# interactiveaudiolab/emphases

Hardware: AMD Instinct MI355X
Metric: utterances/s (10 s @16 kHz) whole-node (higher is better)
Workload: dtype f32; 1 GPU; 64 synthetic 10 s 16 kHz utterances per GPU, conv config, random word alignments, ragged batch with per-utterance (B=1) semantics (BASELINE.json configs[1]); utterances_per_gpu=64, frames_per_gpu=64000, words_per_gpu=1882, conv_tile=64, launch=hipGraph replay, batches_in_flight=2, parallelism=utterance-sharded x1, exchange=none (one rank)

## Files before the change

### emphases_amd/csrc/forward.hip

```cpp
#include "common.h"

using namespace emph;

namespace emph {
__global__ __launch_bounds__(64) void launch_probe_kernel() {}
}

extern "C" {

int emph_launch_probe(void* stream) {
    EMPH_LAUNCH(launch_probe_kernel, dim3(1), dim3(64), 0, static_cast<hipStream_t>(stream));
    return check_launch("emph_launch_probe");
}

int64_t emph_prominence_workspace_floats(int32_t features, int32_t channels,
                                         int64_t ld_frames, int64_t ld_words,
                                         int32_t n_slots) {
    return (static_cast<int64_t>(features) + 2 * channels) * ld_frames +
           static_cast<int64_t>(channels) * (ld_words + n_slots);
}

int emph_prominence_forward(const emph_conv_model* model, const void* audio,
                            int32_t audio_format, const int64_t* seg,
                            const int32_t* frontend_tiles,
// ... 19 lines not shown
                 "emph_prominence_forward: conv_variant %d", m.conv_variant);
    EMPH_REQUIRE(!quad || tile_n == 64, EMPH_ERANGE,
                 "emph_prominence_forward: F(4,3) takes 64-position tiles, not %d", tile_n);
    const int64_t lds_square = quad ? emph_conv_winograd4_lds_bytes(m.channels, m.channels)
                                    : emph_conv_winograd_lds_bytes(m.channels, m.channels);
    const int64_t lds_input = quad ? emph_conv_winograd4_lds_bytes(m.channels, m.features)
                                   : emph_conv_winograd_lds_bytes(m.channels, m.features);
    EMPH_REQUIRE(lds_square <= 160 * 1024 && lds_input <= 160 * 1024, EMPH_ERANGE,
                 "emph_prominence_forward: %d channels do not fit the Winograd kernel's LDS",
                 m.channels);
    const int c = m.channels;
    float* features = workspace;
    float* current = features + static_cast<int64_t>(m.features) * ld_frames;
    float* other = current + static_cast<int64_t>(c) * ld_frames;
    float* words = other + static_cast<int64_t>(c) * ld_frames;
    float* sums = words + static_cast<int64_t>(c) * ld_words;
    const bool fold = word_sums != nullptr && m.encoder_layers > 0;
    EMPH_REQUIRE(!fold || (quad && (m.reduction == EMPH_REDUCE_SUM ||
                                    m.reduction == EMPH_REDUCE_AVERAGE)),
                 EMPH_EINVAL,
                 "emph_prominence_forward: word_sums needs conv_variant 1 and a sum / average "
                 "reduction");

    int status = emph_logmel(audio, audio_format, seg, frontend_tiles, n_frontend_tiles, m.table,
                             m.mel_start, m.mel_count, m.mel_offset, m.mel_values, m.mel_nnz,
                             features, ld_frames, 0, -1, nullptr, nullptr, m.normalize, stream);
    if (status) return status;
    auto conv = [&](const float* in, float* out, const float* pack, const float* bias, int c_in,
                    int activation) {
        return quad ? emph_conv1d_winograd4(in, ld_frames, out, ld_frames, pack, bias, c_in, c,
                                            activation, frame_tiles, n_frame_tiles, stream)
                    : emph_conv1d_winograd(in, ld_frames, out, ld_frames, pack, bias, c_in, c,
                                           activation, frame_tiles, n_frame_tiles, tile_n,
                                           stream);
    };
    const int64_t pack_floats =
        quad ? emph_conv_winograd4_pack_size(c, c) : emph_conv_winograd_pack_size(c, c);
    const bool stack = conv_spans != nullptr && quad && c == 80 && m.features == 80 &&
                       m.encoder_packs == m.input_pack + pack_floats &&
                       m.encoder_biases == m.input_bias + c &&
                       (m.activation == EMPH_ACT_RELU || m.activation == EMPH_ACT_NONE);
    if (stack) {
        const bool composed = m.compose != nullptr && m.encoder_layers >= 1;
        const int skip = composed ? 1 : 0;
        const int total = 1 + m.encoder_layers - skip;
        const int most = emph_conv_stack_max_layers();
        const int groups = (total + most - 1) / most;
        float* buffers[2] = {current, other};
        const float* in = features;
// ... 66 lines not shown
```

### emphases_amd/csrc/frontend.hip

```cpp
#include <math.h>
#include <stdarg.h>

#include "common.h"

namespace emph {

namespace {
thread_local char g_error[512] = "";
}

void set_error(const char* format, ...) {
    va_list args;
    va_start(args, format);
    vsnprintf(g_error, sizeof(g_error), format, args);
    va_end(args);
}

__device__ __forceinline__ void frontend_fence() {
    asm volatile("" ::: "memory");
    __builtin_amdgcn_wave_barrier();
}

__device__ __forceinline__ void frontend_section() { __builtin_amdgcn_sched_barrier(0); }

constexpr float kLn2 = 0.69314718055994530942f;
constexpr int kWaveFrames = 8;
constexpr int kPair = 1;
constexpr int kWavesPerSimd = 3;
constexpr int kTileStride = kWaveFrames + 1;
constexpr int kExRow = 72;
constexpr int kExRowB = 88;
constexpr int kExStepB = 9;
constexpr int kExFloats = 2 * 8 * kExRowB;
__device__ __forceinline__ int spectrum_slot(int k) { return k + 4 * (k >> 5); }
constexpr int kHighBase = 256 + 4 * (256 >> 5);
constexpr int kMagFloats = 560;
constexpr int kWaveFloats = kPair * kExFloats + kMels * kTileStride + kWaveFrames;
constexpr int kRunA = 24;
constexpr int kRunB = 12;

constexpr int kTabWindow = 0;
constexpr int kTabTw1 = 1024;
constexpr int kTabTw2 = kTabTw1 + 2 * 512;
constexpr int kTabTw3 = kTabTw2 + 2 * 64;
constexpr int kTabSize = kTabTw3 + 2 * 514;

typedef float cf __attribute__((ext_vector_type(2)));

template <int STRIDE>
__device__ __forceinline__ void lds_read8(cf (&v)[8], const cf* base) {
    const uint32_t address = static_cast<uint32_t>(reinterpret_cast<uintptr_t>(
        (const __attribute__((address_space(3))) cf*)base));
    asm volatile(
        "ds_read_b64 %0, %8\n\t"
        "ds_read_b64 %1, %8 offset:%9\n\t"
        "ds_read_b64 %2, %8 offset:%10\n\t"
        "ds_read_b64 %3, %8 offset:%11\n\t"
        "ds_read_b64 %4, %8 offset:%12\n\t"
        "ds_read_b64 %5, %8 offset:%13\n\t"
        "ds_read_b64 %6, %8 offset:%14\n\t"
// ... 155 lines not shown
__device__ __forceinline__ void load_edge(const Chunk& chunk, int frame, int p, cf (&s)[8]) {
    const int first = frame * kHop - kPad;
    const int safe = chunk.r_hi > chunk.r_lo ? chunk.r_lo : 0;
#pragma unroll
    for (int q = 0; q < 8; ++q) {
        float pair[2];
#pragma unroll
        for (int h = 0; h < 2; ++h) {
            int r = first + 2 * (p + 64 * q) + h;
            if (r < 0) r = -r;
            if (r >= chunk.length) r = 2 * (chunk.length - 1) - r;
            const bool live = r >= chunk.r_lo && r < chunk.r_hi;
            const int at = live ? r : safe;
            float value = 0.f;
            if (chunk.r_hi > chunk.r_lo)
                value = PCM ? static_cast<float>(static_cast<const int16_t*>(chunk.origin)[at])
                            : static_cast<const float*>(chunk.origin)[at];
            pair[h] = live ? value : 0.f;
        }
        s[q] = {pair[0], pair[1]};
    }
}

template <int MODE, bool PCM>
__global__ __launch_bounds__(256)
__attribute__((amdgpu_waves_per_eu(kWavesPerSimd, kWavesPerSimd))) void frontend_kernel(
    const void* __restrict__ audio, const int64_t* __restrict__ seg,
    const int32_t* __restrict__ tiles, const float* __restrict__ table,
    const int32_t* __restrict__ mel_start, const int32_t* __restrict__ mel_count,
    const int32_t* __restrict__ mel_offset, const float* __restrict__ mel_values,
    int mel_nnz, float* __restrict__ out, int64_t ld, int mel_row, int loud_row,
    float* __restrict__ seg_peak, const float* __restrict__ a_weights,
    int normalize, int n_tiles) {
    constexpr bool kMel = MODE == 0 || MODE == 2;
    constexpr bool kLoud = MODE == 2 || MODE == 3;
    constexpr bool kPeak = MODE == 1;
    constexpr float kPowerFloor = MODE == 0 ? 1e-6f : 0.f;

    extern __shared__ __align__(16) float lds[];
    const int tid = threadIdx.x;
    const int lane = tid & 63;
    const int wave = __builtin_amdgcn_readfirstlane(tid >> 6);
    float* mine = lds + wave * kWaveFloats;
    float* exchange = mine;
    float* tile = exchange + kPair * kExFloats;
    float* loud_tile = tile + kMels * kTileStride;
    float* weights = lds + 4 * kWaveFloats;

    if (kLoud) {
        for (int index = tid; index < kBins; index += 256) weights[index] = a_weights[index];
        __syncthreads();
    }

    const int p = lane;
    const int r1 = lane >> 3;
    const int p0 = lane & 7;
    float window[16];
    cf tw1[8], tw2[8], tw3[4];
#pragma unroll
    for (int q = 0; q < 8; ++q) {
        const float unit = PCM ? 1.f / 32768.f : 1.f;
        window[2 * q] = unit * table[kTabWindow + 2 * (p + 64 * q)];
        window[2 * q + 1] = unit * table[kTabWindow + 2 * (p + 64 * q) + 1];
        tw1[q] = {table[kTabTw1 + 2 * (q * 64 + p)],
                  table[kTabTw1 + 2 * (q * 64 + p) + 1]};
        tw2[q] = {table[kTabTw2 + 2 * (q * 8 + p0)],
                  table[kTabTw2 + 2 * (q * 8 + p0) + 1]};
    }
#pragma unroll
    for (int u = 0; u < 4; ++u) {
        const int k = r1 + 8 * p0 + 64 * u;
        tw3[u] = {table[kTabTw3 + 2 * k + 1], -table[kTabTw3 + 2 * k]};
    }
    auto bin_of = [&](int j) {
        const int k = r1 + 8 * p0 + 64 * (j & 3);
        return j == 8 ? 256 : (j < 4 ? k : 512 - k);
    };

    float weight_a[kRunA], weight_b[kRunB];
    int start_a = 0, start_b = 0;
    if (kMel) {
        const int first_a = mel_start[lane];
        const int count_a = mel_count[lane];
        const int offset_a = mel_offset[lane];
        start_a = first_a & ~3;
#pragma unroll
        for (int j = 0; j < kRunA; ++j) {
            const int index = start_a + j - first_a;
            weight_a[j] = (index >= 0 && index < count_a)
                              ? mel_values[min(max(offset_a + index, 0), mel_nnz - 1)]
                              : 0.f;
        }
        const int row_b = 64 + (lane >> 2);
        const int first_b = mel_start[row_b];
        const int count_b = mel_count[row_b];
        const int offset_b = mel_offset[row_b];
        start_b = (first_b & ~3) + kRunB * (lane & 3);
#pragma unroll
        for (int j = 0; j < kRunB; ++j) {
            const int index = start_b + j - first_b;
            weight_b[j] = (index >= 0 && index < count_b)
                              ? mel_values[min(max(offset_b + index, 0), mel_nnz - 1)]
                              : 0.f;
        }
// ... 142 lines not shown
                    db = fmaxf(db, floor_db) + weights[k];
                    total += static_cast<double>(fmaxf(db, -100.f));
                }
#pragma unroll
                for (int offset = 32; offset > 0; offset >>= 1)
                    total += __shfl_xor(total, offset);
                if (lane == 0) {
                    float value = static_cast<float>(total / 513.);
                    if (normalize) value = (value + 100.f) / 100.f;
                    loud_tile[min(local + f, valid - 1)] = value;
                }
            }
        }

        if (kMel) {
#pragma unroll
            for (int f = 0; f < kPair; ++f) {
                float* mag = exchange + f * kExFloats;
#pragma unroll
                for (int j = 0; j < 8; ++j)
                    mag[bin_of(j)] = __builtin_amdgcn_sqrtf(power[f][j] + (1e-6f - kPowerFloor));
                if (lane == 0)
                    mag[256] = __builtin_amdgcn_sqrtf(power[f][8] + (1e-6f - kPowerFloor));
                if (lane < kMagFloats - kBins) mag[kBins + lane] = 0.f;
            }
            frontend_fence();
#pragma unroll
            for (int f = 0; f < kPair; ++f) {
                const float* mag = exchange + f * kExFloats;
                const int column = min(local + f, valid - 1);
                float acc = 0.f;
#pragma unroll
                for (int piece = 0; piece < kRunA / 4; ++piece) {
                    const float4 four =
                        *reinterpret_cast<const float4*>(mag + start_a + 4 * piece);
                    acc = fmaf(weight_a[4 * piece], four.x, acc);
                    acc = fmaf(weight_a[4 * piece + 1], four.y, acc);
                    acc = fmaf(weight_a[4 * piece + 2], four.z, acc);
                    acc = fmaf(weight_a[4 * piece + 3], four.w, acc);
                }
                float value = kLn2 * __builtin_amdgcn_logf(fmaxf(acc, 1e-5f));
                if (normalize) value = fmaf(value, 0.1f, 1.f);
                tile[lane * kTileStride + column] = value;
                acc = 0.f;
#pragma unroll
                for (int piece = 0; piece < kRunB / 4; ++piece) {
                    const float4 four =
                        *reinterpret_cast<const float4*>(mag + start_b + 4 * piece);
                    acc = fmaf(weight_b[4 * piece], four.x, acc);
                    acc = fmaf(weight_b[4 * piece + 1], four.y, acc);
                    acc = fmaf(weight_b[4 * piece + 2], four.z, acc);
// ... 70 lines not shown
            0.5f * static_cast<float>(0.5 - 0.5 * cos(two_pi * n / kFft));
    for (int r = 0; r < 8; ++r)
        for (int p = 0; p < 64; ++p) {
            const double angle = -two_pi * (p * r) / 512.;
            host_table[kTabTw1 + 2 * (r * 64 + p)] = static_cast<float>(cos(angle));
            host_table[kTabTw1 + 2 * (r * 64 + p) + 1] =
                static_cast<float>(sin(angle));
        }
    for (int t = 0; t < 8; ++t)
        for (int p0 = 0; p0 < 8; ++p0) {
            const double angle = -two_pi * (p0 * t) / 64.;
            host_table[kTabTw2 + 2 * (t * 8 + p0)] = static_cast<float>(cos(angle));
            host_table[kTabTw2 + 2 * (t * 8 + p0) + 1] =
                static_cast<float>(sin(angle));
        }
    for (int k = 0; k < 514; ++k) {
        const double angle = -two_pi * k / 1024.;
        host_table[kTabTw3 + 2 * k] = static_cast<float>(cos(angle));
        host_table[kTabTw3 + 2 * k + 1] = static_cast<float>(sin(angle));
    }
    return EMPH_OK;
}

int emph_logmel(const void* audio, int32_t audio_format, const int64_t* seg,
                const int32_t* tiles, int32_t n_tiles, const float* table,
                const int32_t* mel_start, const int32_t* mel_count,
                const int32_t* mel_offset, const float* mel_values, int32_t mel_nnz,
                float* out, int64_t ld, int32_t mel_row, int32_t loud_row,
                const float* seg_peak, const float* a_weights, int32_t normalize,
                void* stream) {
    if (n_tiles == 0) return EMPH_OK;
    const bool mel = mel_row >= 0, loud = loud_row >= 0;
    EMPH_REQUIRE(audio && seg && tiles && table && out, EMPH_EINVAL,
                 "emph_logmel: null pointer");
    EMPH_REQUIRE(audio_format == EMPH_AUDIO_F32 || audio_format == EMPH_AUDIO_PCM16,
                 EMPH_EINVAL, "emph_logmel: unknown audio format %d", audio_format);
    EMPH_REQUIRE(mel || loud, EMPH_EINVAL, "emph_logmel: no output row selected");
    EMPH_REQUIRE(!mel || (mel_start && mel_count && mel_offset && mel_values),
                 EMPH_EINVAL, "emph_logmel: mel basis is null");
    EMPH_REQUIRE(!mel || (mel_nnz > 0 && mel_nnz <= 8192), EMPH_ERANGE,
                 "emph_logmel: mel_nnz %d out of range", mel_nnz);
    EMPH_REQUIRE(!loud || (seg_peak && a_weights), EMPH_EINVAL,
                 "emph_logmel: loudness needs seg_peak and a_weights");
    const size_t lds = frontend_lds_bytes(loud);
    hipStream_t s = static_cast<hipStream_t>(stream);
    float* peak = const_cast<float*>(seg_peak);
    const bool pcm = audio_format == EMPH_AUDIO_PCM16;
#define EMPH_FRONTEND(MODE, PCM)                                                          \
    do {                                                                                  \
        auto kernel = frontend_kernel<MODE, PCM>;                                         \
        static LdsReservation reserved;                                                   \
        if (int status = reserve_lds(reserved, reinterpret_cast<const void*>(kernel),     \
                                     lds, "emph_logmel"))                                 \
            return status;                                                                \
        EMPH_LAUNCH(kernel, dim3(frontend_grid(n_tiles)), dim3(256), lds, s, audio, seg,  \
                    tiles, table, mel_start, mel_count, mel_offset, mel_values, mel_nnz,  \
                    out, ld, mel_row, loud_row, peak, a_weights, normalize, n_tiles);     \
    } while (0)
    if (mel && loud) {
        if (pcm) EMPH_FRONTEND(2, true); else EMPH_FRONTEND(2, false);
    } else if (mel) {
        if (pcm) EMPH_FRONTEND(0, true); else EMPH_FRONTEND(0, false);
    } else {
        if (pcm) EMPH_FRONTEND(3, true); else EMPH_FRONTEND(3, false);
    }
    return check_launch("emph_logmel");
}

int emph_frontend_peak(const void* audio, int32_t audio_format, const int64_t* seg,
                       const int32_t* tiles, int32_t n_tiles, const float* table,
                       float* seg_peak, void* stream) {
    if (n_tiles == 0) return EMPH_OK;
    EMPH_REQUIRE(audio && seg && tiles && table && seg_peak, EMPH_EINVAL,
                 "emph_frontend_peak: null pointer");
    EMPH_REQUIRE(audio_format == EMPH_AUDIO_F32 || audio_format == EMPH_AUDIO_PCM16,
                 EMPH_EINVAL, "emph_frontend_peak: unknown audio format %d", audio_format);
    const size_t lds = frontend_lds_bytes(false);
    hipStream_t s = static_cast<hipStream_t>(stream);
    const int32_t* mel_start = nullptr;
    const int32_t* mel_count = nullptr;
    const int32_t* mel_offset = nullptr;
    const float* mel_values = nullptr;
    const float* a_weights = nullptr;
    float* out = nullptr;
    float* peak = seg_peak;
    const int64_t ld = 0;
    const int mel_nnz = 0, mel_row = -1, loud_row = -1, normalize = 0;
    if (audio_format == EMPH_AUDIO_PCM16) EMPH_FRONTEND(1, true); else EMPH_FRONTEND(1, false);
    return check_launch("emph_frontend_peak");
}
#undef EMPH_FRONTEND

}
```

### emphases_amd/engine.py

```python
import contextlib
import functools
import os
import ctypes
import threading

import numpy as np
import torch

from . import config as cfg
from . import melbasis
from . import runtime
from . import weights as weights_module

FRONTEND_BLOCK = None
PRECISIONS = {'f32': (0, 0, 0), 'bf16x3': (2, 32, 3), 'bf16x3_fast': (2, 32, 2),
              'bf16x6': (0, 3, 3)}
ATTENTION_BLOCK = 64
ATTENTION_GROUP = 256
GROUPED_FROM = ATTENTION_GROUP // 2
FUSED_WORDS = 64
EVERYTHING = 1 << 30
SHORT, LONG = (0, GROUPED_FROM - 1), (GROUPED_FROM, EVERYTHING)
FEW_WORDS, MANY_WORDS = (0, FUSED_WORDS), (FUSED_WORDS + 1, EVERYTHING)
WORD_TILE = 16
# ... 22 lines not shown
                f'head dimension {head_dim} (channels {channels} / heads '
                f'{config.heads}) not in {{32, 40, 64}}')
    elif config.layers > 16:
        raise ValueError(f'{config.layers} convolution layers > 16')
    if config.architecture == 'convolution' or not config.has_decoder:
        if channels < 16 or channels % 16:
            raise ValueError(
                f'channels {channels} not a multiple of 16 in 16..128 (the '
                'fused word stage of this configuration)')
        if config.decoder_kernel_size not in (1, 3, 5):
            raise ValueError(
                f'decoder kernel size {config.decoder_kernel_size} not in '
                '{1, 3, 5} (the fused word stage of this configuration)')
        layers = config.layers if config.has_decoder else 0
        if runtime.library().emph_word_decoder_block(
                layers, config.decoder_kernel_size,
                config.decoder_kernel_size) < 16:
            raise ValueError(
                f'{layers} decoder layers of kernel size '
                f'{config.decoder_kernel_size}: the receptive field is too '
                "wide for the fused word stage's 64-word window")


def a_weighting():
    frequencies = np.fft.rfftfreq(n=1024, d=1.0 / 8000)
    f_sq = frequencies ** 2.0
    const = np.array([12194.217, 20.598997, 107.65265, 737.86223]) ** 2.0
    with np.errstate(divide='ignore'):
        weights = 2.0 + 20.0 * (
            np.log10(const[0]) + 2 * np.log10(f_sq)
            - np.log10(f_sq + const[0]) - np.log10(f_sq + const[1])
            - 0.5 * np.log10(f_sq + const[2])
            - 0.5 * np.log10(f_sq + const[3]))
    return (np.maximum(-80.0, weights) - cfg.REF_DB).astype(np.float32)


class _Conv:

    def __init__(self, weight, bias, device, winograd=False):
        weight = np.asarray(weight, dtype=np.float32)
        if weight.ndim == 2:
            weight = weight[:, :, None]
        self.c_out, self.c_in, self.kernel_size = weight.shape
        self.weight = weight
        self.pack = torch.from_numpy(runtime.conv_pack(weight)).to(device)
        self.winograd = None
# ... 33 lines not shown
        self.conv_tile = conv_tile
        self.timers = None
        self._workspace = {}
        self._staging = {}
        self.lock = threading.RLock()
        self.split_tile = int(os.environ.get('EMPHASES_SPLIT_TILE', 16))
        if self.split_tile not in (16, 32):
            raise ValueError('EMPHASES_SPLIT_TILE must be 16 or 32')
        self.max_columns = SPLIT16_COLUMNS if (
            config.architecture == 'transformer' and self.linear_pieces and
            self.split_tile == 16) else KERNEL_COLUMNS
        state = weights_module.load(state, config)
        self.state = state
        dev = self.device
        to = lambda a: torch.from_numpy(np.ascontiguousarray(a)).to(dev)

        self.table = to(runtime.frontend_table())
        basis = melbasis.default()
        self.mel_start = to(basis.row_start)
        self.mel_count = to(basis.row_count)
        self.mel_offset = to(basis.row_offset)
        self.mel_values = to(basis.values)
        self.mel_nnz = int(basis.values.size)
        self.a_weights = to(a_weighting())

        self.input_layer = _Conv(
            state['input_layer.weight'], state['input_layer.bias'], dev,
            winograd)
        self.frame_encoder = self._stack('frame_encoder')
        self.word_decoder = self._stack('word_decoder') \
            if config.has_decoder else None
        self.output_weight = to(state['output_layer.weight'])
        self.output_bias = to(state['output_layer.bias'])
        self.fused_words = config.architecture == 'convolution' or \
            not config.has_decoder
        self.word_block = WORD_TILE
        if self.fused_words:
            layers = self.word_decoder if config.has_decoder else []
            self.decoder_layers = len(layers)
            self.decoder_packs = torch.from_numpy(np.concatenate([
                runtime.word_decoder_pack(l.weight) for l in layers])).to(dev) \
                if layers else None
            self.decoder_biases = torch.cat([l.bias for l in layers]) \
                if layers else None
            self.word_block = int(self.lib.emph_word_decoder_block(
                self.decoder_layers, config.decoder_kernel_size,
# ... 93 lines not shown
                if encoder else torch.zeros(1, device=self.device)
        pointer = lambda t: None if t is None else t.data_ptr()
        return runtime.ConvModel(
            channels=config.channels, features=config.num_features,
            encoder_layers=len(encoder), decoder_layers=self.decoder_layers,
            decoder_kernel_size=config.decoder_kernel_size,
            activation=runtime.ACTIVATIONS[config.activation],
            reduction=runtime.REDUCTIONS[config.downsample_method],
            post=runtime.POSTPROCESS[config.loss],
            normalize=int(config.normalize), mel_nnz=self.mel_nnz,
            conv_variant=int(self.quad),
            table=pointer(self.table), mel_start=pointer(self.mel_start),
            mel_count=pointer(self.mel_count),
            mel_offset=pointer(self.mel_offset),
            mel_values=pointer(self.mel_values),
            input_pack=pointer(input_pack),
            input_bias=pointer(input_bias),
            encoder_packs=pointer(self._encoder_packs),
            encoder_biases=pointer(self._encoder_biases),
            decoder_packs=pointer(self.decoder_packs),
            decoder_biases=pointer(self.decoder_biases),
            out_weight=pointer(self.output_weight),
            out_bias=pointer(self.output_bias),
            compose=pointer(self._compose_pack if self.stack else None))

    def _stack(self, prefix):
        config, state, dev = self.config, self.state, self.device
        layers = []
        if config.architecture == 'convolution':
            for i in range(config.layers):
                layers.append(_Conv(
                    state[f'{prefix}.{2 * i}.weight'],
                    state[f'{prefix}.{2 * i}.bias'], dev,
                    self.winograd and prefix == 'frame_encoder'))
            return layers
        channels = config.channels
        to = lambda a: torch.from_numpy(np.ascontiguousarray(a)).to(dev)
        for i in range(config.layers):
            p = f'{prefix}.model.layers.{i}.'
            in_w = state[p + 'self_attn.in_proj_weight']
            in_b = state[p + 'self_attn.in_proj_bias']
            block = None
            square = (channels, channels)
            if channels in (64, 80) and all(
                    tuple(state[p + name].shape) == square for name in (
                        'self_attn.out_proj.weight', 'linear1.weight',
                        'linear2.weight')):
# ... 284 lines not shown
            with self._timed('pitch_rows'):
                runtime.check(self.lib.emph_pitch_rows(
                    tracks[0].data_ptr(), tracks[1].data_ptr(),
                    out.data_ptr(), plan.ld_frames, pitch_row,
                    periodicity_row, int(config.normalize),
                    float(np.log2(np.float32(cfg.FMIN))),
                    float(np.log2(np.float32(cfg.FMAX))), runtime.stream()),
                    'emph_pitch_rows')
        tiles, size = meta[('tiles', runtime.AXIS_FRAMES, FRONTEND_BLOCK)]
        count = size // runtime.TILE_FIELDS
        table = meta['table'][0]
        peak = None
        if config.loudness_feature:
            peak = torch.zeros(
                len(plan), dtype=torch.float32, device=self.device)
            with self._timed('frontend_peak'):
                runtime.check(self.lib.emph_frontend_peak(
                    audio.data_ptr(), audio_format(audio), table.data_ptr(),
                    tiles.data_ptr(),
                    count, self.table.data_ptr(), peak.data_ptr(),
                    runtime.stream()), 'emph_frontend_peak')
        if mel_row >= 0 or loud_row >= 0:
            with self._timed('frontend_logmel'):
                runtime.check(self.lib.emph_logmel(
                    audio.data_ptr(), audio_format(audio), table.data_ptr(),
                    tiles.data_ptr(),
                    count, self.table.data_ptr(), self.mel_start.data_ptr(),
                    self.mel_count.data_ptr(), self.mel_offset.data_ptr(),
                    self.mel_values.data_ptr(), self.mel_nnz, out.data_ptr(),
                    plan.ld_frames, mel_row, loud_row,
                    None if peak is None else peak.data_ptr(),
                    self.a_weights.data_ptr(), int(config.normalize),
                    runtime.stream()), 'emph_logmel')
        return out

    def _transformer(self, layers, x, ld, plan, meta, axis, block, tag,
                     key_counts=None, positioned=False, select=()):
        config = self.config
        channels = config.channels
        if block > 32 and ('tiles', axis, 32) + select in meta:
            block = 32
        att_tiles, att_size = meta[('tiles', axis, ATTENTION_BLOCK) + select]
        att_count = att_size // runtime.TILE_FIELDS
        if att_count == 0:
            return x
        counts = plan.frames if axis == runtime.AXIS_FRAMES else plan.words
        if len(counts) and int(counts.max()) > cfg.MAX_POSITIONS:
            raise RuntimeError(
                f'a chunk of {int(counts.max())} positions exceeds the '
                f'{cfg.MAX_POSITIONS}-entry positional encoding; pass a '
                'smaller batch_size')
        if not positioned:
            with self._timed('add_position'):
# ... 658 lines not shown
```

### emphases_amd/runtime.py

```python
import ctypes
import os

import numpy as np
import torch

HERE = os.path.dirname(os.path.abspath(__file__))
LIBRARY_PATH = os.path.join(HERE, 'libemphases_hip.so')
ABI_VERSION = 41

SEG_FIELDS = 8
TILE_FIELDS = 4
(SEG_AUDIO_OFF, SEG_AUDIO_LEN, SEG_START, SEG_LENGTH, SEG_FRAME_OFF,
 SEG_FRAMES, SEG_WORD_OFF, SEG_WORDS) = range(8)
AXIS_FRAMES, AXIS_WORDS = 0, 1
AXIS_DECODER = 2
ACTIVATIONS = {None: 0, 'none': 0, 'relu': 1, 'gelu': 2, 'silu': 3,
               'leaky_relu': 4}
REDUCTIONS = {'sum': 0, 'average': 1, 'max': 2, 'center': 3}
POSTPROCESS = {None: 0, 'bce': 1, 'mse': 2}
BCE_FORMS = {'bce': 0, 'mse': 1}
UPSAMPLE_METHODS = {'linear': 0, 'nearest': 1}
AUDIO_F32, AUDIO_PCM16 = 0, 1
SPREAD_IDENTITY, SPREAD_LOG2 = 0, 1
(METRIC_COUNT, METRIC_BCE, METRIC_SQUARED_ERROR, METRIC_COVARIANCE,
 METRIC_SUM_PREDICTED, METRIC_SUMSQ_PREDICTED, METRIC_SUM_TARGET,
 METRIC_SUMSQ_TARGET, METRIC_FIELDS) = range(9)

_c = ctypes
_ptr, _i32, _i64, _f32 = _c.c_void_p, _c.c_int32, _c.c_int64, _c.c_float

SIGNATURES = {
    'emph_abi_version': (_c.c_int, []),
    'emph_last_error': (_c.c_char_p, []),
    'emph_launch_probe': (_c.c_int, [_ptr]),
    'emph_launch_timer_begin': (_c.c_int, [_i32]),
    'emph_launch_timer_count': (_i32, []),
    'emph_launch_timer_end': (_c.c_int, [_ptr, _i32, _ptr]),
    'emph_frontend_table_size': (_i64, []),
    'emph_frontend_table_fill': (_c.c_int, [_ptr]),
    'emph_frontend_block': (_i32, []),
    'emph_logmel': (_c.c_int, [
        _ptr, _i32, _ptr, _ptr, _i32, _ptr, _ptr, _ptr, _ptr, _ptr, _i32, _ptr,
        _i64, _i32, _i32, _ptr, _ptr, _i32, _ptr]),
    'emph_frontend_peak': (_c.c_int, [
        _ptr, _i32, _ptr, _ptr, _i32, _ptr, _ptr, _ptr]),
    'emph_host_gather': (_c.c_int, [_ptr, _ptr, _ptr, _i32, _ptr, _i32]),
    'emph_resample': (_c.c_int, [
        _ptr, _i32, _ptr, _i32, _i64, _ptr, _i32, _i32, _i32, _ptr, _ptr]),
    'emph_pitch_rows': (_c.c_int, [
        _ptr, _ptr, _ptr, _i64, _i32, _i32, _i32, _f32, _f32, _ptr]),
    'emph_conv_pack_size': (_i64, [_i32, _i32, _i32]),
    'emph_conv_pack': (_c.c_int, [_ptr, _i32, _i32, _i32, _ptr]),
    'emph_conv1d': (_c.c_int, [
        _ptr, _i64, _ptr, _i64, _ptr, _ptr, _i32, _i32, _i32, _i32, _ptr, _i32,
        _i32, _i32, _ptr]),
    'emph_conv_winograd_pack_size': (_i64, [_i32, _i32]),
    'emph_conv_winograd_lds_bytes': (_i64, [_i32, _i32]),
    'emph_conv_winograd_pack': (_c.c_int, [_ptr, _i32, _i32, _ptr]),
    'emph_conv1d_winograd': (_c.c_int, [
        _ptr, _i64, _ptr, _i64, _ptr, _ptr, _i32, _i32, _i32, _ptr, _i32, _i32,
        _ptr]),
    'emph_conv_winograd4_pack_size': (_i64, [_i32, _i32]),
    'emph_conv_winograd4_lds_bytes': (_i64, [_i32, _i32]),
    'emph_conv_winograd4_pack': (_c.c_int, [_ptr, _i32, _i32, _ptr]),
    'emph_conv1d_winograd4': (_c.c_int, [
        _ptr, _i64, _ptr, _i64, _ptr, _ptr, _i32, _i32, _i32, _ptr, _i32,
# ... 258 lines not shown
    def count(self):
        return int(library().emph_launch_timer_count())

    def __exit__(self, kind, value, trace):
        durations = np.zeros(self.capacity, dtype=np.float32)
        seen = _i32(0)
        status = library().emph_launch_timer_end(
            durations.ctypes.data, self.capacity, _c.byref(seen))
        if kind is None:
            check(status, 'emph_launch_timer_end')
        self.launches = int(seen.value)
        self.microseconds = durations[:min(self.launches, self.capacity)]
        return False


def frontend_table():
    lib = library()
    table = np.zeros(lib.emph_frontend_table_size(), dtype=np.float32)
    check(lib.emph_frontend_table_fill(table.ctypes.data),
          'emph_frontend_table_fill')
    return table


def linear_chain_pack(weight, natural):
    lib = library()
    weight = np.ascontiguousarray(weight, dtype=np.float32)
    channels = weight.shape[0]
    assert weight.shape == (channels, channels)
    pack = np.zeros(lib.emph_linear_chain_pack_size(channels),
                    dtype=np.float32)
    check(lib.emph_linear_chain_pack(
        weight.ctypes.data, channels, int(natural), pack.ctypes.data),
        'emph_linear_chain_pack')
    return pack


def word_decoder_tiles(counts, offsets, layers, kernel_size, out_kernel_size):
    lib = library()
    counts = np.ascontiguousarray(counts, dtype=np.int64)
    offsets = np.ascontiguousarray(offsets, dtype=np.int64)
    arguments = (counts.ctypes.data, offsets.ctypes.data, len(counts),
                 int(layers), int(kernel_size), int(out_kernel_size))
    total = lib.emph_word_decoder_tiles(*arguments, None)
    if total < 0:
        raise ValueError('emph_word_decoder_tiles: bad decoder shape')
    tiles = np.zeros((total, TILE_FIELDS), dtype=np.int32)
# ... 6 lines not shown
    lib = library()
    names = ('self_attn.in_proj_weight', 'self_attn.in_proj_bias',
             'self_attn.out_proj.weight', 'self_attn.out_proj.bias',
             'linear1.weight', 'linear1.bias', 'linear2.weight', 'linear2.bias',
             'norm1.weight', 'norm1.bias', 'norm2.weight', 'norm2.bias')
    arrays = [np.ascontiguousarray(state[prefix + name], dtype=np.float32)
              for name in names]
    pack = np.zeros(lib.emph_word_transformer_pack_size(channels, heads),
                    dtype=np.float32)
    check(lib.emph_word_transformer_pack(
        *[array.ctypes.data for array in arrays], channels, heads,
        pack.ctypes.data), 'emph_word_transformer_pack')
    return pack


class ConvModel(_c.Structure):
    _fields_ = [(name, _i32) for name in (
        'channels', 'features', 'encoder_layers', 'decoder_layers',
        'decoder_kernel_size', 'activation', 'reduction', 'post',
        'normalize', 'mel_nnz', 'conv_variant')] + [(name, _ptr) for name in (
            'table', 'mel_start', 'mel_count', 'mel_offset', 'mel_values',
            'input_pack', 'input_bias', 'encoder_packs', 'encoder_biases',
            'decoder_packs', 'decoder_biases', 'out_weight', 'out_bias',
            'compose')]


class WordSumTables(_c.Structure):
    _fields_ = [(name, _ptr) for name in (
        'slot_map', 'terms', 'first', 'lengths')] + [('n_slots', _i32)]


def word_decoder_pack(weight):
    lib = library()
    weight = np.ascontiguousarray(weight, dtype=np.float32)
    channels, c_in, kernel_size = weight.shape
    assert channels == c_in
    pack = np.zeros(
        lib.emph_word_decoder_pack_size(channels, kernel_size),
        dtype=np.float32)
    check(lib.emph_word_decoder_pack(
        weight.ctypes.data, channels, kernel_size, pack.ctypes.data),
        'emph_word_decoder_pack')
    return pack


def conv_compose_pack(w0, b0, w1, b1):
    lib = library()
# ... 82 lines not shown
```

### include/emphases_hip.h

```cpp
#ifndef EMPHASES_HIP_H
#define EMPHASES_HIP_H

#include <stdint.h>

#ifdef __cplusplus
extern "C" {
#endif

#define EMPH_ABI_VERSION 41

enum {
    EMPH_SEG_AUDIO_OFF = 0,
    EMPH_SEG_AUDIO_LEN = 1,
    EMPH_SEG_START = 2,
    EMPH_SEG_LENGTH = 3,
    EMPH_SEG_FRAME_OFF = 4,
    EMPH_SEG_FRAMES = 5,
    EMPH_SEG_WORD_OFF = 6,
    EMPH_SEG_WORDS = 7,
    EMPH_SEG_FIELDS = 8
};

enum { EMPH_AXIS_FRAMES = 0, EMPH_AXIS_WORDS = 1 };

enum {
    EMPH_TILE_SEGMENT = 0,
    EMPH_TILE_FIRST = 1,
    EMPH_TILE_OFFSET = 2,
    EMPH_TILE_COUNT = 3,
    EMPH_TILE_FIELDS = 4
};

// ... 77 lines not shown
int64_t emph_plan_word_sums(const int64_t* frames, const int64_t* frame_off,
                            const int64_t* words, int32_t n_segments,
                            const int64_t* word_columns, const int64_t* bounds,
                            int64_t total_words, const int64_t* restarts,
                            int64_t n_restarts, int64_t ld_frames,
                            int64_t ld_words, int32_t* slot_map, int32_t* first,
                            int32_t* lengths, int32_t* terms, int64_t capacity,
                            int32_t* n_slots);


int64_t emph_frontend_table_size(void);

int32_t emph_frontend_block(void);

int emph_frontend_table_fill(float* host_table);

int emph_logmel(const void* audio, int32_t audio_format, const int64_t* seg,
                const int32_t* tiles, int32_t n_tiles, const float* table,
                const int32_t* mel_start, const int32_t* mel_count,
                const int32_t* mel_offset, const float* mel_values,
                int32_t mel_nnz, float* out, int64_t ld, int32_t mel_row,
                int32_t loud_row, const float* seg_peak,
                const float* a_weights, int32_t normalize, void* stream);

int emph_frontend_peak(const void* audio, int32_t audio_format,
                       const int64_t* seg, const int32_t* tiles,
                       int32_t n_tiles, const float* table, float* seg_peak,
                       void* stream);

int emph_resample(const void* audio, int32_t audio_format, const int64_t* table,
                  int32_t n_utterances, int64_t most_samples,
                  const float* kernel, int32_t orig, int32_t fresh,
                  int32_t width, float* out, void* stream);

int emph_pitch_rows(const float* pitch, const float* periodicity, float* out,
                    int64_t ld, int32_t pitch_row, int32_t periodicity_row,
                    int32_t normalize, float logfmin, float logfmax,
                    void* stream);


int64_t emph_conv_pack_size(int32_t c_out, int32_t c_in, int32_t kernel_size);

int emph_conv_pack(const float* host_weight, int32_t c_out, int32_t c_in,
                   int32_t kernel_size, float* host_pack);

int emph_conv1d(const float* x, int64_t ldx, float* y, int64_t ldy,
// ... 271 lines not shown
    int32_t encoder_layers;
    int32_t decoder_layers;
    int32_t decoder_kernel_size;
    int32_t activation;
    int32_t reduction;
    int32_t post;
    int32_t normalize;
    int32_t mel_nnz;
    int32_t conv_variant;
    const float* table;
    const int32_t* mel_start;
    const int32_t* mel_count;
    const int32_t* mel_offset;
    const float* mel_values;
    const float* input_pack;
    const float* input_bias;
    const float* encoder_packs;
    const float* encoder_biases;
    const float* decoder_packs;
    const float* decoder_biases;
    const float* out_weight;
    const float* out_bias;
    const float* compose;
} emph_conv_model;

typedef struct emph_word_sum_tables {
    const int32_t* slot_map;
    const int32_t* terms;
    const int32_t* first;
    const int32_t* lengths;
    int32_t n_slots;
} emph_word_sum_tables;

int64_t emph_prominence_workspace_floats(int32_t features, int32_t channels,
                                         int64_t ld_frames, int64_t ld_words,
                                         int32_t n_slots);

int emph_prominence_forward(const emph_conv_model* model, const void* audio,
                            int32_t audio_format, const int64_t* seg,
                            const int32_t* frontend_tiles,
                            int32_t n_frontend_tiles,
                            const int32_t* frame_tiles, int32_t n_frame_tiles,
                            int32_t tile_n, const int32_t* word_tiles,
                            int32_t n_word_tiles, const int32_t* bounds,
                            const int32_t* word_segment, int64_t ld_frames,
                            int64_t ld_words, float* workspace, float* logits,
// ... 116 lines not shown
```

Measured before the change: 463,800 utterances/s.

## Precompute a bank-conflict-aware quad plan for the mel filterbank projection

Adds a host-built plan that splits the sparse mel basis into 4-bin quads spread evenly across the 64 lanes, each lane reading float4 magnitudes and writing per-row partial sums into LDS slots. A random-swap search assigns runs to lanes to minimise LDS bank conflicts, and a second pass reduces up to four partials per mel row before the log. The aim is to replace the uneven per-row runs (weight_a/weight_b) with balanced vector reads. In exchange it costs extra LDS per wave, more registers for the per-lane weights, and an extra fence and reduction pass per frame.

```diff
diff --git a/emphases_amd/csrc/forward.hip b/emphases_amd/csrc/forward.hip
--- a/emphases_amd/csrc/forward.hip
+++ b/emphases_amd/csrc/forward.hip
@@ -65,9 +65,10 @@
                  "emph_prominence_forward: word_sums needs conv_variant 1 and a sum / average "
                  "reduction");
 
-    int status = emph_logmel(audio, audio_format, seg, frontend_tiles, n_frontend_tiles, m.table,
-                             m.mel_start, m.mel_count, m.mel_offset, m.mel_values, m.mel_nnz,
-                             features, ld_frames, 0, -1, nullptr, nullptr, m.normalize, stream);
+    int status = emph_logmel_planned(audio, audio_format, seg, frontend_tiles, n_frontend_tiles,
+                                     m.table, m.mel_start, m.mel_count, m.mel_offset,
+                                     m.mel_values, m.mel_nnz, m.mel_plan, features, ld_frames, 0,
+                                     -1, nullptr, nullptr, m.normalize, stream);
     if (status) return status;
     auto conv = [&](const float* in, float* out, const float* pack, const float* bias, int c_in,
                     int activation) {
diff --git a/emphases_amd/csrc/frontend.hip b/emphases_amd/csrc/frontend.hip
--- a/emphases_amd/csrc/frontend.hip
+++ b/emphases_amd/csrc/frontend.hip
@@ -1,5 +1,6 @@
 #include <math.h>
 #include <stdarg.h>
+#include <string.h>
 
 #include "common.h"
 
@@ -35,7 +36,20 @@
 __device__ __forceinline__ int spectrum_slot(int k) { return k + 4 * (k >> 5); }
 constexpr int kHighBase = 256 + 4 * (256 >> 5);
 constexpr int kMagFloats = 560;
-constexpr int kWaveFloats = kPair * kExFloats + kMels * kTileStride + kWaveFrames;
+constexpr int kQuads = 5;
+constexpr int kPartSlots = 4;
+constexpr int kPartSpare = kMels * kPartSlots;
+constexpr int kPartFloats = kPartSpare + 64;
+constexpr int kWaveFloats =
+    kPair * kExFloats + kMels * kTileStride + kWaveFrames + kPartFloats;
+static_assert(kWaveFloats % 4 == 0 && (kWaveFloats - kPartFloats) % 4 == 0,
+              "the partial slots are read 16 bytes at a time");
+constexpr int kPlanRead = 0;
+constexpr int kPlanWrite = kPlanRead + kQuads * 64;
+constexpr int kPlanWeight = kPlanWrite + kQuads * 64;
+constexpr int kPlanRestart = kPlanWeight + 4 * kQuads * 64;
+constexpr int kPlanTail = kPlanRestart + 64;
+constexpr int kPlanSize = kPlanTail + 64;
 constexpr int kRunA = 24;
 constexpr int kRunB = 12;
 
@@ -237,14 +251,15 @@
     }
 }
 
-template <int MODE, bool PCM>
+template <int MODE, bool PCM, bool QUADS>
 __global__ __launch_bounds__(256)
 __attribute__((amdgpu_waves_per_eu(kWavesPerSimd, kWavesPerSimd))) void frontend_kernel(
     const void* __restrict__ audio, const int64_t* __restrict__ seg,
     const int32_t* __restrict__ tiles, const float* __restrict__ table,
     const int32_t* __restrict__ mel_start, const int32_t* __restrict__ mel_count,
     const int32_t* __restrict__ mel_offset, const float* __restrict__ mel_values,
-    int mel_nnz, float* __restrict__ out, int64_t ld, int mel_row, int loud_row,
+    int mel_nnz, const uint32_t* __restrict__ mel_plan, float* __restrict__ out, int64_t ld,
+    int mel_row, int loud_row,
     float* __restrict__ seg_peak, const float* __restrict__ a_weights,
     int normalize, int n_tiles) {
     constexpr bool kMel = MODE == 0 || MODE == 2;
@@ -260,6 +275,7 @@
     float* exchange = mine;
     float* tile = exchange + kPair * kExFloats;
     float* loud_tile = tile + kMels * kTileStride;
+    float* parts = loud_tile + kWaveFrames;
     float* weights = lds + 4 * kWaveFloats;
 
     if (kLoud) {
@@ -294,7 +310,27 @@
 
     float weight_a[kRunA], weight_b[kRunB];
     int start_a = 0, start_b = 0;
-    if (kMel) {
+    float quad_weight[4 * kQuads];
+    int quad_read[kQuads], quad_write[kQuads];
+    uint64_t quad_restart[kQuads];
+    bool zero_tail = true;
+    if (kMel && QUADS) {
+        zero_tail = __builtin_amdgcn_readfirstlane(static_cast<int>(mel_plan[kPlanTail])) != 0;
+        const uint32_t restarts = mel_plan[kPlanRestart + lane];
+#pragma unroll
+        for (int j = 0; j < kQuads; ++j) {
+            quad_read[j] = static_cast<int>(mel_plan[kPlanRead + 64 * j + lane]);
+            quad_write[j] = static_cast<int>(mel_plan[kPlanWrite + 64 * j + lane]);
+            quad_restart[j] = __builtin_amdgcn_ballot_w64(((restarts >> j) & 1u) != 0);
+#pragma unroll
+            for (int i = 0; i < 4; ++i)
+                quad_weight[4 * j + i] =
+                    __uint_as_float(mel_plan[kPlanWeight + 64 * (4 * j + i) + lane]);
+        }
+#pragma unroll
+        for (int index = lane; index < kPartFloats; index += 64) parts[index] = 0.f;
+        frontend_fence();
+    } else if (kMel) {
         const int first_a = mel_start[lane];
         const int count_a = mel_count[lane];
         const int offset_a = mel_offset[lane];
@@ -483,11 +519,46 @@
                     mag[bin_of(j)] = __builtin_amdgcn_sqrtf(power[f][j] + (1e-6f - kPowerFloor));
                 if (lane == 0)
                     mag[256] = __builtin_amdgcn_sqrtf(power[f][8] + (1e-6f - kPowerFloor));
-                if (lane < kMagFloats - kBins) mag[kBins + lane] = 0.f;
+                if (zero_tail && lane < kMagFloats - kBins) mag[kBins + lane] = 0.f;
             }
             frontend_fence();
 #pragma unroll
-            for (int f = 0; f < kPair; ++f) {
+            for (int f = 0; f < (QUADS ? kPair : 0); ++f) {
+                const float* mag = exchange + f * kExFloats;
+                const int column = min(local + f, valid - 1);
+                float acc = 0.f;
+                float4 four[kQuads];
+#pragma unroll
+                for (int j = 0; j < kQuads; ++j)
+                    four[j] = *reinterpret_cast<const float4*>(mag + quad_read[j]);
+#pragma unroll
+                for (int j = 0; j < kQuads; ++j) {
+                    if (j)
+                        asm("v_cndmask_b32_e64 %0, %1, 0, %2"
+                            : "=v"(acc) : "v"(acc), "s"(quad_restart[j]));
+                    acc = fmaf(quad_weight[4 * j], four[j].x, acc);
+                    acc = fmaf(quad_weight[4 * j + 1], four[j].y, acc);
+                    acc = fmaf(quad_weight[4 * j + 2], four[j].z, acc);
+                    acc = fmaf(quad_weight[4 * j + 3], four[j].w, acc);
+                    parts[quad_write[j]] = acc;
+                }
+                frontend_fence();
+#pragma unroll
+                for (int pass = 0; pass < 2; ++pass) {
+                    const int m = 64 * pass + lane;
+                    if (m < kMels) {
+                        const float4 slot =
+                            *reinterpret_cast<const float4*>(parts + kPartSlots * m);
+                        const float sum = ((slot.x + slot.y) + slot.z) + slot.w;
+                        float value = kLn2 * __builtin_amdgcn_logf(fmaxf(sum, 1e-5f));
+                        if (normalize) value = fmaf(value, 0.1f, 1.f);
+                        tile[m * kTileStride + column] = value;
+                    }
+                }
+                frontend_fence();
+            }
+#pragma unroll
+            for (int f = 0; f < (QUADS ? 0 : kPair); ++f) {
                 const float* mag = exchange + f * kExFloats;
                 const int column = min(local + f, valid - 1);
                 float acc = 0.f;
@@ -604,6 +675,171 @@
     return EMPH_OK;
 }
 
+int64_t emph_frontend_mel_plan_size(void) { return kPlanSize; }
+
+int emph_frontend_mel_plan_fill(const int32_t* mel_start, const int32_t* mel_count,
+                                const int32_t* mel_offset, const float* mel_values,
+                                int32_t mel_nnz, uint32_t* host_plan, int32_t* counts) {
+    EMPH_REQUIRE(mel_start && mel_count && mel_offset && mel_values && host_plan, EMPH_EINVAL,
+                 "emph_frontend_mel_plan_fill: null pointer");
+    struct Piece {
+        int row, bin;
+        float weight[4];
+    };
+    static_assert(kPartSlots == 4, "a row's slots are one 16-byte read");
+    constexpr int kMost = 64 * kQuads;
+    Piece pieces[kMost];
+    int n = 0;
+    for (int row = 0; row < kMels; ++row) {
+        const int start = mel_start[row], count = mel_count[row], offset = mel_offset[row];
+        EMPH_REQUIRE(start >= 0 && count >= 0 && start + count <= kBins && offset >= 0 &&
+                         offset + count <= mel_nnz,
+                     EMPH_EINVAL, "emph_frontend_mel_plan_fill: row %d: run [%d, %d) at %d of %d",
+                     row, start, start + count, offset, mel_nnz);
+        int low = 0, high = count;
+        while (low < high && mel_values[offset + low] == 0.f) ++low;
+        while (high > low && mel_values[offset + high - 1] == 0.f) --high;
+        if (low == high) continue;
+        const int first = start + low, last = start + high - 1;
+        for (int bin = first & ~3; bin <= last; bin += 4) {
+            EMPH_REQUIRE(n < kMost, EMPH_ERANGE,
+                         "emph_frontend_mel_plan_fill: the basis has more than %d quads "
+                         "(%d per lane)", kMost, kQuads);
+            Piece& piece = pieces[n++];
+            piece.row = row;
+            piece.bin = bin;
+            for (int i = 0; i < 4; ++i)
+                piece.weight[i] = bin + i >= first && bin + i <= last
+                                      ? mel_values[offset + bin + i - start] : 0.f;
+        }
+    }
+    static_assert(((kBins - 1) | 3) < kMagFloats, "a quad stays inside the magnitude buffer");
+    int begin_of[65];
+    int most_quads = 0;
+    for (int most = 3; most <= kQuads; most += kQuads - 3) {
+        int at = 0;
+        most_quads = 0;
+        for (int run = 0; run < 64; ++run) {
+            begin_of[run] = at;
+            int partials = 0;
+            const int even = most == kQuads ? (n + 63) / 64 : kQuads;
+            while (at < n && at - begin_of[run] < even) {
+                const bool opens = at == begin_of[run] || pieces[at].row != pieces[at - 1].row;
+                if (opens && partials == most) break;
+                partials += opens;
+                ++at;
+            }
+            if (at - begin_of[run] > most_quads) most_quads = at - begin_of[run];
+        }
+        begin_of[64] = at;
+        if (at == n) break;
+    }
+    auto chunk_of = [&](int run, int j) {
+        const int mine = begin_of[run + 1] - begin_of[run];
+        return mine ? pieces[begin_of[run] + (j < mine ? j : mine - 1)].bin >> 2 : 0;
+    };
+    auto group_of = [](int lane) {
+        const int low = lane & 31;
+        const bool first = low < 4 || (low >= 12 && low < 16) || (low >= 20 && low < 28);
+        return 2 * (lane >> 5) + (first ? 0 : 1);
+    };
+    int run_of[64];
+    for (int lane = 0; lane < 64; ++lane) run_of[lane] = lane;
+    auto cycles_of = [&](int group) {
+        int cycles = 0;
+        for (int j = 0; j < kQuads; ++j) {
+            int chunks[16], count = 0, worst = 0;
+            for (int lane = 0; lane < 64; ++lane)
+                if (group_of(lane) == group) chunks[count++] = chunk_of(run_of[lane], j);
+            for (int a = 0; a < count; ++a) {
+                int same_bank = 1;
+                for (int c = 0; c < count; ++c) {
+                    if ((chunks[c] & 15) != (chunks[a] & 15) || chunks[c] == chunks[a]) continue;
+                    bool seen = false;
+                    for (int d = 0; d < c; ++d) seen = seen || chunks[d] == chunks[c];
+                    same_bank += !seen;
+                }
+                if (same_bank > worst) worst = same_bank;
+            }
+            cycles += worst;
+        }
+        return cycles;
+    };
+    int cycles[4];
+    for (int group = 0; group < 4; ++group) cycles[group] = cycles_of(group);
+    uint32_t state = 12345u;
+    for (int trial = 0; trial < 40000; ++trial) {
+        state = state * 1103515245u + 12345u;
+        const int a = (state >> 8) & 63;
+        state = state * 1103515245u + 12345u;
+        const int c = (state >> 8) & 63;
+        const int ga = group_of(a), gc = group_of(c);
+        if (ga == gc) continue;
+        if (cycles[0] + cycles[1] + cycles[2] + cycles[3] == 4 * kQuads) break;
+        int swap = run_of[a];
+        run_of[a] = run_of[c];
+        run_of[c] = swap;
+        const int now_a = cycles_of(ga), now_c = cycles_of(gc);
+        if (now_a + now_c <= cycles[ga] + cycles[gc]) {
+            cycles[ga] = now_a;
+            cycles[gc] = now_c;
+        } else {
+            run_of[c] = run_of[a];
+            run_of[a] = swap;
+        }
+    }
+    int lane_of[64];
+    for (int lane = 0; lane < 64; ++lane) lane_of[run_of[lane]] = lane;
+    bool tail = false;
+    for (int index = 0; index < n; ++index) tail = tail || pieces[index].bin + 3 >= kBins;
+    for (int index = 0; index < 64; ++index) host_plan[kPlanTail + index] = tail;
+    int row_lanes[kMels] = {0};
+    int most_partials = 0, most_lanes = 0;
+    for (int run = 0; run < 64; ++run) {
+        const int lane = lane_of[run];
+        const int begin = begin_of[run];
+        const int mine = begin_of[run + 1] - begin;
+        uint32_t restarts = 0;
+        int partials = 0;
+        for (int j = 0; j < kQuads; ++j) {
+            const bool live = j < mine;
+            const Piece* piece = mine ? &pieces[begin + (live ? j : mine - 1)] : nullptr;
+            host_plan[kPlanRead + 64 * j + lane] = piece ? piece->bin : 0;
+            for (int i = 0; i < 4; ++i) {
+                const float weight = live ? piece->weight[i] : 0.f;
+                uint32_t bits;
+                memcpy(&bits, &weight, sizeof(bits));
+                host_plan[kPlanWeight + 64 * (4 * j + i) + lane] = bits;
+            }
+            if (live && j > 0 && piece->row != pieces[begin + j - 1].row) restarts |= 1u << j;
+            const bool closes = mine && (j == kQuads - 1 ||
+                                         (j + 1 < mine && pieces[begin + j + 1].row != piece->row));
+            int where = kPartSpare + lane;
+            if (closes) {
+                const int slot = row_lanes[piece->row]++;
+                EMPH_REQUIRE(slot < kPartSlots, EMPH_ERANGE,
+                             "emph_frontend_mel_plan_fill: row %d is spread over more than "
+                             "%d lanes", piece->row, kPartSlots);
+                where = kPartSlots * piece->row + slot;
+                ++partials;
+            }
+            host_plan[kPlanWrite + 64 * j + lane] = where;
+        }
+        host_plan[kPlanRestart + lane] = restarts;
+        if (partials > most_partials) most_partials = partials;
+    }
+    for (int row = 0; row < kMels; ++row)
+        if (row_lanes[row] > most_lanes) most_lanes = row_lanes[row];
+    if (counts) {
+        counts[0] = n;
+        counts[1] = most_quads;
+        counts[2] = most_partials;
+        counts[3] = most_lanes;
+        counts[4] = cycles[0] + cycles[1] + cycles[2] + cycles[3];
+    }
+    return EMPH_OK;
+}
+
 int emph_logmel(const void* audio, int32_t audio_format, const int64_t* seg,
                 const int32_t* tiles, int32_t n_tiles, const float* table,
                 const int32_t* mel_start, const int32_t* mel_count,
@@ -611,6 +847,18 @@
                 float* out, int64_t ld, int32_t mel_row, int32_t loud_row,
                 const float* seg_peak, const float* a_weights, int32_t normalize,
                 void* stream) {
+    return emph_logmel_planned(audio, audio_format, seg, tiles, n_tiles, table, mel_start,
+                               mel_count, mel_offset, mel_values, mel_nnz, nullptr, out, ld,
+                               mel_row, loud_row, seg_peak, a_weights, normalize, stream);
+}
+
+int emph_logmel_planned(const void* audio, int32_t audio_format, const int64_t* seg,
+                        const int32_t* tiles, int32_t n_tiles, const float* table,
+                        const int32_t* mel_start, const int32_t* mel_count,
+                        const int32_t* mel_offset, const float* mel_values, int32_t mel_nnz,
+                        const uint32_t* mel_plan, float* out, int64_t ld, int32_t mel_row,
+                        int32_t loud_row, const float* seg_peak, const float* a_weights,
+                        int32_t normalize, void* stream) {
     if (n_tiles == 0) return EMPH_OK;
     const bool mel = mel_row >= 0, loud = loud_row >= 0;
     EMPH_REQUIRE(audio && seg && tiles && table && out, EMPH_EINVAL,
@@ -628,23 +876,28 @@
     hipStream_t s = static_cast<hipStream_t>(stream);
     float* peak = const_cast<float*>(seg_peak);
     const bool pcm = audio_format == EMPH_AUDIO_PCM16;
-#define EMPH_FRONTEND(MODE, PCM)                                                          \
+#define EMPH_FRONTEND(MODE, PCM, QUADS)                                                   \
     do {                                                                                  \
-        auto kernel = frontend_kernel<MODE, PCM>;                                         \
+        auto kernel = frontend_kernel<MODE, PCM, QUADS>;                                       \
         static LdsReservation reserved;                                                   \
         if (int status = reserve_lds(reserved, reinterpret_cast<const void*>(kernel),     \
                                      lds, "emph_logmel"))                                 \
             return status;                                                                \
         EMPH_LAUNCH(kernel, dim3(frontend_grid(n_tiles)), dim3(256), lds, s, audio, seg,  \
                     tiles, table, mel_start, mel_count, mel_offset, mel_values, mel_nnz,  \
-                    out, ld, mel_row, loud_row, peak, a_weights, normalize, n_tiles);     \
+                    mel_plan, out, ld, mel_row, loud_row, peak, a_weights, normalize,     \
+                    n_tiles);                                                             \
     } while (0)
-    if (mel && loud) {
-        if (pcm) EMPH_FRONTEND(2, true); else EMPH_FRONTEND(2, false);
+    if (mel && loud && mel_plan) {
+        if (pcm) EMPH_FRONTEND(2, true, true); else EMPH_FRONTEND(2, false, true);
+    } else if (mel && loud) {
+        if (pcm) EMPH_FRONTEND(2, true, false); else EMPH_FRONTEND(2, false, false);
+    } else if (mel && mel_plan) {
+        if (pcm) EMPH_FRONTEND(0, true, true); else EMPH_FRONTEND(0, false, true);
     } else if (mel) {
-        if (pcm) EMPH_FRONTEND(0, true); else EMPH_FRONTEND(0, false);
+        if (pcm) EMPH_FRONTEND(0, true, false); else EMPH_FRONTEND(0, false, false);
     } else {
-        if (pcm) EMPH_FRONTEND(3, true); else EMPH_FRONTEND(3, false);
+        if (pcm) EMPH_FRONTEND(3, true, false); else EMPH_FRONTEND(3, false, false);
     }
     return check_launch("emph_logmel");
 }
@@ -667,8 +920,10 @@
     float* out = nullptr;
     float* peak = seg_peak;
     const int64_t ld = 0;
+    const uint32_t* mel_plan = nullptr;
     const int mel_nnz = 0, mel_row = -1, loud_row = -1, normalize = 0;
-    if (audio_format == EMPH_AUDIO_PCM16) EMPH_FRONTEND(1, true); else EMPH_FRONTEND(1, false);
+    if (audio_format == EMPH_AUDIO_PCM16) EMPH_FRONTEND(1, true, false);
+    else EMPH_FRONTEND(1, false, false);
     return check_launch("emph_frontend_peak");
 }
 #undef EMPH_FRONTEND
diff --git a/emphases_amd/engine.py b/emphases_amd/engine.py
--- a/emphases_amd/engine.py
+++ b/emphases_amd/engine.py
@@ -68,6 +68,14 @@
                 "wide for the fused word stage's 64-word window")
 
 
+@functools.lru_cache(maxsize=None)
+def _default_mel_plan():
+    basis = melbasis.default()
+    plan, _ = runtime.frontend_mel_plan(
+        basis.row_start, basis.row_count, basis.row_offset, basis.values)
+    return plan
+
+
 def a_weighting():
     frequencies = np.fft.rfftfreq(n=1024, d=1.0 / 8000)
     f_sq = frequencies ** 2.0
@@ -147,6 +155,13 @@
         self.mel_offset = to(basis.row_offset)
         self.mel_values = to(basis.values)
         self.mel_nnz = int(basis.values.size)
+        self.mel_plan = None
+        if os.environ.get('EMPHASES_MEL_PLAN', '1') != '0' and \
+                config.architecture == 'convolution' and \
+                config.downsample_method in ('sum', 'average'):
+            mel_plan = _default_mel_plan()
+            self.mel_plan = None if mel_plan is None else \
+                to(mel_plan.view(np.int32))
         self.a_weights = to(a_weighting())
 
         self.input_layer = _Conv(
@@ -286,7 +301,8 @@
             decoder_biases=pointer(self.decoder_biases),
             out_weight=pointer(self.output_weight),
             out_bias=pointer(self.output_bias),
-            compose=pointer(self._compose_pack if self.stack else None))
+            compose=pointer(self._compose_pack if self.stack else None),
+            mel_plan=pointer(self.mel_plan))
 
     def _stack(self, prefix):
         config, state, dev = self.config, self.state, self.device
@@ -617,13 +633,14 @@
                     runtime.stream()), 'emph_frontend_peak')
         if mel_row >= 0 or loud_row >= 0:
             with self._timed('frontend_logmel'):
-                runtime.check(self.lib.emph_logmel(
+                runtime.check(self.lib.emph_logmel_planned(
                     audio.data_ptr(), audio_format(audio), table.data_ptr(),
                     tiles.data_ptr(),
                     count, self.table.data_ptr(), self.mel_start.data_ptr(),
                     self.mel_count.data_ptr(), self.mel_offset.data_ptr(),
-                    self.mel_values.data_ptr(), self.mel_nnz, out.data_ptr(),
-                    plan.ld_frames, mel_row, loud_row,
+                    self.mel_values.data_ptr(), self.mel_nnz,
+                    None if self.mel_plan is None else self.mel_plan.data_ptr(),
+                    out.data_ptr(), plan.ld_frames, mel_row, loud_row,
                     None if peak is None else peak.data_ptr(),
                     self.a_weights.data_ptr(), int(config.normalize),
                     runtime.stream()), 'emph_logmel')
diff --git a/emphases_amd/runtime.py b/emphases_amd/runtime.py
--- a/emphases_amd/runtime.py
+++ b/emphases_amd/runtime.py
@@ -6,7 +6,7 @@
 
 HERE = os.path.dirname(os.path.abspath(__file__))
 LIBRARY_PATH = os.path.join(HERE, 'libemphases_hip.so')
-ABI_VERSION = 41
+ABI_VERSION = 42
 
 SEG_FIELDS = 8
 TILE_FIELDS = 4
@@ -42,6 +42,12 @@
     'emph_logmel': (_c.c_int, [
         _ptr, _i32, _ptr, _ptr, _i32, _ptr, _ptr, _ptr, _ptr, _ptr, _i32, _ptr,
         _i64, _i32, _i32, _ptr, _ptr, _i32, _ptr]),
+    'emph_frontend_mel_plan_size': (_i64, []),
+    'emph_frontend_mel_plan_fill': (_c.c_int, [
+        _ptr, _ptr, _ptr, _ptr, _i32, _ptr, _ptr]),
+    'emph_logmel_planned': (_c.c_int, [
+        _ptr, _i32, _ptr, _ptr, _i32, _ptr, _ptr, _ptr, _ptr, _ptr, _i32, _ptr,
+        _ptr, _i64, _i32, _i32, _ptr, _ptr, _i32, _ptr]),
     'emph_frontend_peak': (_c.c_int, [
         _ptr, _i32, _ptr, _ptr, _i32, _ptr, _ptr, _ptr]),
     'emph_host_gather': (_c.c_int, [_ptr, _ptr, _ptr, _i32, _ptr, _i32]),
@@ -346,6 +352,25 @@
     return table
 
 
+ERANGE = -2
+
+
+def frontend_mel_plan(start, count, offset, values):
+    lib = library()
+    start, count, offset = (np.ascontiguousarray(a, dtype=np.int32)
+                            for a in (start, count, offset))
+    values = np.ascontiguousarray(values, dtype=np.float32)
+    plan = np.zeros(lib.emph_frontend_mel_plan_size(), dtype=np.uint32)
+    counts = np.zeros(5, dtype=np.int32)
+    status = lib.emph_frontend_mel_plan_fill(
+        start.ctypes.data, count.ctypes.data, offset.ctypes.data,
+        values.ctypes.data, values.size, plan.ctypes.data, counts.ctypes.data)
+    if status == ERANGE:
+        return None, None
+    check(status, 'emph_frontend_mel_plan_fill')
+    return plan, counts
+
+
 def linear_chain_pack(weight, natural):
     lib = library()
     weight = np.ascontiguousarray(weight, dtype=np.float32)
@@ -398,7 +423,7 @@
             'table', 'mel_start', 'mel_count', 'mel_offset', 'mel_values',
             'input_pack', 'input_bias', 'encoder_packs', 'encoder_biases',
             'decoder_packs', 'decoder_biases', 'out_weight', 'out_bias',
-            'compose')]
+            'compose', 'mel_plan')]
 
 
 class WordSumTables(_c.Structure):
diff --git a/include/emphases_hip.h b/include/emphases_hip.h
--- a/include/emphases_hip.h
+++ b/include/emphases_hip.h
@@ -7,7 +7,7 @@
 extern "C" {
 #endif
 
-#define EMPH_ABI_VERSION 41
+#define EMPH_ABI_VERSION 42
 
 enum {
     EMPH_SEG_AUDIO_OFF = 0,
@@ -131,6 +131,19 @@
                 int32_t mel_nnz, float* out, int64_t ld, int32_t mel_row,
                 int32_t loud_row, const float* seg_peak,
                 const float* a_weights, int32_t normalize, void* stream);
+
+int64_t emph_frontend_mel_plan_size(void);
+int emph_frontend_mel_plan_fill(const int32_t* mel_start, const int32_t* mel_count,
+                                const int32_t* mel_offset, const float* mel_values,
+                                int32_t mel_nnz, uint32_t* host_plan, int32_t* counts);
+int emph_logmel_planned(const void* audio, int32_t audio_format, const int64_t* seg,
+                        const int32_t* tiles, int32_t n_tiles, const float* table,
+                        const int32_t* mel_start, const int32_t* mel_count,
+                        const int32_t* mel_offset, const float* mel_values,
+                        int32_t mel_nnz, const uint32_t* mel_plan, float* out,
+                        int64_t ld, int32_t mel_row, int32_t loud_row,
+                        const float* seg_peak, const float* a_weights,
+                        int32_t normalize, void* stream);
 
 int emph_frontend_peak(const void* audio, int32_t audio_format,
                        const int64_t* seg, const int32_t* tiles,
@@ -448,6 +461,7 @@
     const float* out_weight;
     const float* out_bias;
     const float* compose;
+    const uint32_t* mel_plan;
 } emph_conv_model;
 
 typedef struct emph_word_sum_tables {
```

New measurement: 469,400 utterances/s (median of 6 runs). +1.2%, better.
